# ryantd/tf-operator

Measured on AMD Instinct MI355X. Metric: samples/sec (1-worker TFJob), higher is better.
Workload: dtype bf16

## Files before the change

### csrc/hip/optim.hip

```cpp
#include "toa_common.h"

#include <algorithm>

template <bool BF16>
__global__ __launch_bounds__(256) void sumsq_partial_kernel(const void* __restrict__ x, int64_t n,
                                                            float* __restrict__ partial) {
  __shared__ float red[4];
  float acc = 0.f;
  const int64_t n8 = n / 8;
  for (int64_t i = blockIdx.x * (int64_t)blockDim.x + threadIdx.x; i < n8;
       i += (int64_t)gridDim.x * blockDim.x) {
    float f[8];
    if (BF16) {
      unpack8(ld16((const bf16_t*)x + i * 8), f);
    } else {
      f32x4 a = *((const f32x4*)x + 2 * i), b = *((const f32x4*)x + 2 * i + 1);
      f[0] = a[0]; f[1] = a[1]; f[2] = a[2]; f[3] = a[3];
      f[4] = b[0]; f[5] = b[1]; f[6] = b[2]; f[7] = b[3];
    }
#pragma unroll
    for (int j = 0; j < 8; ++j) acc = fmaf(f[j], f[j], acc);
  }
  if (blockIdx.x == 0) {
    for (int64_t i = n8 * 8 + threadIdx.x; i < n; i += blockDim.x) {
// ... 150 lines not shown
  const float ns = norm_sq[0];
  const bool bad = (__float_as_uint(ns) & 0x7f800000u) == 0x7f800000u;
  const int f = (bad || (limit > 0.f && sqrtf(ns) * grad_scale > limit)) ? 1 : 0;
  flag[0] = f;
  skipped[0] += f;
}

extern "C" int toa_adamw_guard(const float* norm_sq, float grad_scale, float limit, int* flag, int* skipped,
                               hipStream_t stream) {
  if (norm_sq == nullptr || flag == nullptr || skipped == nullptr) return (int)hipErrorInvalidValue;
  hipLaunchKernelGGL(adamw_guard_kernel, dim3(1), dim3(1), 0, stream, norm_sq, grad_scale, limit, flag, skipped);
  return (int)hipGetLastError();
}

__device__ __forceinline__ int guard_step(int step, const int* skipped, float b1, float b2, float& inv_bc1,
                                          float& inv_sqrt_bc2) {
  const int sk = skipped[0];
  if (sk != 0) {
    const float st = (float)(step - sk);
    inv_bc1 = 1.f / (1.f - powf(b1, st));
    inv_sqrt_bc2 = 1.f / sqrtf(1.f - powf(b2, st));
  }
  return step - sk;
}

template <bool GRAD_BF16, bool NT, typename MT = float, bool GUARD = false>
__global__ __launch_bounds__(256) void adamw_flat_kernel(float* __restrict__ master, bf16_t* __restrict__ param,
                                                         void* __restrict__ grad, int zero_grad, MT* __restrict__ m,
                                                         MT* __restrict__ v, int64_t n8, float lr, float b1,
                                                         float b2, float eps, float wd, float inv_bc1,
                                                         float inv_sqrt_bc2, float grad_scale,
                                                         const float* __restrict__ norm_sq, float max_norm,
                                                         const int* __restrict__ step_dev, int step, int64_t base,
                                                         uint32_t seed, const int* __restrict__ flag,
                                                         const int* __restrict__ skipped) {
  constexpr bool MB = sizeof(MT) == 2;
  if constexpr (GUARD) {
    if (flag[0] != 0) {
      if (zero_grad) {
        const int64_t nz = GRAD_BF16 ? n8 : 2 * n8;
        for (int64_t i = blockIdx.x * (int64_t)blockDim.x + threadIdx.x; i < nz; i += (int64_t)gridDim.x * blockDim.x)
          *((u32x4*)grad + i) = u32x4{0, 0, 0, 0};
      }
      return;
    }
    step = guard_step(step, skipped, b1, b2, inv_bc1, inv_sqrt_bc2);
  }
  const float scale = adam_prologue(b1, b2, grad_scale, norm_sq, max_norm, step_dev, inv_bc1, inv_sqrt_bc2);
  const float omb1 = 1.f - b1, omb2 = 1.f - b2, lrwd = lr * wd;
  const uint32_t key = MB ? sr_key(step_dev != nullptr ? step_dev[0] : step, seed) : 0u;
  for (int64_t i = blockIdx.x * (int64_t)blockDim.x + threadIdx.x; i < n8;
       i += (int64_t)gridDim.x * blockDim.x) {
    float g[8], p[8], mm[8], vv[8];
    if (GRAD_BF16) {
      unpack8(ld_s((const u32x4*)grad + i, NT), g);
      if (zero_grad) st16((bf16_t*)grad + i * 8, u32x4{0, 0, 0, 0});
    } else {
      f32x4 a = ld_s((const f32x4*)grad + 2 * i, NT), b = ld_s((const f32x4*)grad + 2 * i + 1, NT);
      g[0] = a[0]; g[1] = a[1]; g[2] = a[2]; g[3] = a[3];
      g[4] = b[0]; g[5] = b[1]; g[6] = b[2]; g[7] = b[3];
      if (zero_grad) {
        *((f32x4*)grad + 2 * i) = f32x4{0.f, 0.f, 0.f, 0.f};
        *((f32x4*)grad + 2 * i + 1) = f32x4{0.f, 0.f, 0.f, 0.f};
      }
    }
    f32x4* pm = (f32x4*)master + 2 * i;
    f32x4 p0 = ld_s(pm, NT), p1 = ld_s(pm + 1, NT);
    if constexpr (MB) {
      u32x4* mv = (u32x4*)m + i;
      u32x4* vvp = (u32x4*)v + i;
      const u32x4 mb = ld_s(mv, NT), vb = ld_s(vvp, NT);
      unpack8(mb, mm);
      unpack8(vb, vv);
#pragma unroll
      for (int j = 0; j < 4; ++j) {
        p[j] = p0[j]; p[j + 4] = p1[j];
      }
#pragma unroll
      for (int j = 0; j < 8; ++j)
        adam_elem(g[j], p[j], mm[j], vv[j], scale, b1, b2, omb1, omb2, lr, lrwd, eps, inv_bc1, inv_sqrt_bc2);
#pragma unroll
      for (int j = 0; j < 4; ++j) {
        p0[j] = p[j]; p1[j] = p[j + 4];
      }
      u32x4 mo, vo;
      sr_pack8(mm, vv, base + 8 * i, key, mo, vo);
      st_s(pm, p0, NT); st_s(pm + 1, p1, NT);
      st_s(mv, mo, NT);
      st_s(vvp, vo, NT);
    } else {
      f32x4* mv = (f32x4*)m + 2 * i;
      f32x4* vvp = (f32x4*)v + 2 * i;
      f32x4 m0 = ld_s(mv, NT), m1 = ld_s(mv + 1, NT), v0 = ld_s(vvp, NT), v1 = ld_s(vvp + 1, NT);
#pragma unroll
      for (int j = 0; j < 4; ++j) {
        p[j] = p0[j]; p[j + 4] = p1[j];
        mm[j] = m0[j]; mm[j + 4] = m1[j];
        vv[j] = v0[j]; vv[j + 4] = v1[j];
      }
#pragma unroll
      for (int j = 0; j < 8; ++j)
        adam_elem(g[j], p[j], mm[j], vv[j], scale, b1, b2, omb1, omb2, lr, lrwd, eps, inv_bc1, inv_sqrt_bc2);
#pragma unroll
      for (int j = 0; j < 4; ++j) {
        p0[j] = p[j]; p1[j] = p[j + 4];
        m0[j] = mm[j]; m1[j] = mm[j + 4];
        v0[j] = vv[j]; v1[j] = vv[j + 4];
      }
      st_s(pm, p0, NT); st_s(pm + 1, p1, NT);
      st_s(mv, m0, NT); st_s(mv + 1, m1, NT);
      st_s(vvp, v0, NT); st_s(vvp + 1, v1, NT);
    }
    if (param != nullptr) st_s((u32x4*)param + i, pack8(p), NT);
  }
}

template <typename MT = float, bool GUARD = false>
__global__ __launch_bounds__(256) void adamw_wt_kernel(float* __restrict__ master, bf16_t* __restrict__ param,
                                                       bf16_t* __restrict__ grad, int zero_grad,
                                                       MT* __restrict__ m, MT* __restrict__ v,
                                                       bf16_t* __restrict__ wt, int64_t ldt, int R, int C, float lr,
                                                       float b1, float b2, float eps, float wd, float inv_bc1,
                                                       float inv_sqrt_bc2, float grad_scale,
                                                       const float* __restrict__ norm_sq, float max_norm, int step,
                                                       int64_t base, uint32_t seed, const int* __restrict__ flag,
                                                       const int* __restrict__ skipped) {
  constexpr bool MB = sizeof(MT) == 2;
  __shared__ u32x4 tile[128 * 16];
  if constexpr (GUARD) {
    if (flag[0] != 0) {
      if (zero_grad) {
        const int64_t nz = (int64_t)R * C / 8;
        for (int64_t i = blockIdx.x * (int64_t)blockDim.x + threadIdx.x; i < nz; i += (int64_t)gridDim.x * blockDim.x)
          st16(grad + i * 8, u32x4{0, 0, 0, 0});
      }
      return;
    }
    step = guard_step(step, skipped, b1, b2, inv_bc1, inv_sqrt_bc2);
  }
  const float scale = adam_prologue(b1, b2, grad_scale, norm_sq, max_norm, nullptr, inv_bc1, inv_sqrt_bc2);
  const float omb1 = 1.f - b1, omb2 = 1.f - b2, lrwd = lr * wd;
  const uint32_t key = MB ? sr_key(step, seed) : 0u;
  const int tid = threadIdx.x;
  const int lr_ = tid >> 4, lc = tid & 15;
  const int a = tid & 15, bq = tid >> 4;
  const int tiles_c = C >> 7;
  const int64_t ntiles = (int64_t)(R >> 7) * tiles_c;
  for (int64_t t = blockIdx.x; t < ntiles; t += gridDim.x) {
    const int tr = (int)(t / tiles_c), tc = (int)(t - (int64_t)tr * tiles_c);
    const int64_t r0 = (int64_t)tr * 128, c0 = (int64_t)tc * 128;
    __syncthreads();
#pragma unroll 1
    for (int pp = 0; pp < 8; pp += 2) {
      u32x4 gb[2], mb[2], vb[2];
      f32x4 pv[2][2], mv[2][2], vv[2][2];
      int64_t e8[2];
#pragma unroll
      for (int q = 0; q < 2; ++q) {
        const int r = lr_ + 16 * (pp + q);
        e8[q] = ((r0 + r) * C + c0) / 8 + lc;
        gb[q] = ld_s((const u32x4*)grad + e8[q], true);
        pv[q][0] = ld_s((const f32x4*)master + 2 * e8[q], true);
        pv[q][1] = ld_s((const f32x4*)master + 2 * e8[q] + 1, true);
        if constexpr (MB) {
          mb[q] = ld_s((const u32x4*)m + e8[q], true);
          vb[q] = ld_s((const u32x4*)v + e8[q], true);
        } else {
          mv[q][0] = ld_s((const f32x4*)m + 2 * e8[q], true);
          mv[q][1] = ld_s((const f32x4*)m + 2 * e8[q] + 1, true);
          vv[q][0] = ld_s((const f32x4*)v + 2 * e8[q], true);
          vv[q][1] = ld_s((const f32x4*)v + 2 * e8[q] + 1, true);
        }
      }
#pragma unroll
      for (int q = 0; q < 2; ++q) {
        const int r = lr_ + 16 * (pp + q);
        float g[8], p[8];
        unpack8(gb[q], g);
        if (zero_grad) st16(grad + e8[q] * 8, u32x4{0, 0, 0, 0});
        if constexpr (MB) {
          float t[8];
          unpack8(mb[q], t);
          mv[q][0] = f32x4{t[0], t[1], t[2], t[3]};
          mv[q][1] = f32x4{t[4], t[5], t[6], t[7]};
          unpack8(vb[q], t);
          vv[q][0] = f32x4{t[0], t[1], t[2], t[3]};
          vv[q][1] = f32x4{t[4], t[5], t[6], t[7]};
        }
#pragma unroll
        for (int h = 0; h < 2; ++h)
#pragma unroll
          for (int j = 0; j < 4; ++j) {
            float pp_ = pv[q][h][j], mm = mv[q][h][j], vq = vv[q][h][j];
            adam_elem(g[4 * h + j], pp_, mm, vq, scale, b1, b2, omb1, omb2, lr, lrwd, eps, inv_bc1, inv_sqrt_bc2);
            pv[q][h][j] = pp_;
            mv[q][h][j] = mm;
            vv[q][h][j] = vq;
            p[4 * h + j] = pp_;
          }
        st_s((f32x4*)master + 2 * e8[q], pv[q][0], true);
        st_s((f32x4*)master + 2 * e8[q] + 1, pv[q][1], true);
        if constexpr (MB) {
          const float mf[8] = {mv[q][0][0], mv[q][0][1], mv[q][0][2], mv[q][0][3],
                               mv[q][1][0], mv[q][1][1], mv[q][1][2], mv[q][1][3]};
          const float vf[8] = {vv[q][0][0], vv[q][0][1], vv[q][0][2], vv[q][0][3],
                               vv[q][1][0], vv[q][1][1], vv[q][1][2], vv[q][1][3]};
          u32x4 mo, vo;
          sr_pack8(mf, vf, base + 8 * e8[q], key, mo, vo);
          st_s((u32x4*)m + e8[q], mo, true);
          st_s((u32x4*)v + e8[q], vo, true);
        } else {
          st_s((f32x4*)m + 2 * e8[q], mv[q][0], true);
          st_s((f32x4*)m + 2 * e8[q] + 1, mv[q][1], true);
          st_s((f32x4*)v + 2 * e8[q], vv[q][0], true);
          st_s((f32x4*)v + 2 * e8[q] + 1, vv[q][1], true);
        }
        const u32x4 pk = pack8(p);
        st_s((u32x4*)param + e8[q], pk, true);
        tile[r * 16 + (lc ^ ((r >> 3) & 15))] = pk;
      }
    }
    __syncthreads();
    u32x4 in[8], out[8];
#pragma unroll
    for (int i = 0; i < 8; ++i) in[i] = tile[(8 * a + i) * 16 + (bq ^ a)];
    tr8x8(in, out);
    bf16_t* d = wt + (c0 + 8 * bq) * ldt + r0 + 8 * a;
#pragma unroll
    for (int j = 0; j < 8; ++j) __builtin_nontemporal_store(out[j], (u32x4*)(d + j * ldt));
  }
}

template <typename MT, bool GUARD = false>
static int adamw_wt_launch(float* master, bf16_t* param, bf16_t* grad, int zero_grad, MT* m, MT* v, bf16_t* wt,
                           int64_t ldt, int R, int C, float lr, float beta1, float beta2, float eps,
                           float weight_decay, int step, float grad_scale, const float* norm_sq, float max_norm,
                           int64_t base, uint32_t seed, hipStream_t stream, const int* flag = nullptr,
                           const int* skipped = nullptr) {
  if (GUARD && (flag == nullptr || skipped == nullptr)) return (int)hipErrorInvalidValue;
  if (R <= 0 || C <= 0 || R % 128 || C % 128 || ldt < R || ldt % 8 || ((uintptr_t)master & 15) ||
      ((uintptr_t)m & 15) || ((uintptr_t)v & 15) || ((uintptr_t)grad & 15) || ((uintptr_t)param & 15) ||
      ((uintptr_t)wt & 15) || step < 1 || base < 0 || base % 8)
    return (int)hipErrorInvalidValue;
  const float inv_bc1 = 1.f / (1.f - powf(beta1, (float)step));
  const float inv_sqrt_bc2 = 1.f / sqrtf(1.f - powf(beta2, (float)step));
  const int64_t tiles = (int64_t)(R / 128) * (C / 128);
  const int grid = (int)(tiles < 16384 ? tiles : 16384);
  hipLaunchKernelGGL((adamw_wt_kernel<MT, GUARD>), dim3(grid), dim3(256), 0, stream, master, param, grad, zero_grad,
                     m, v, wt, ldt, R, C, lr, beta1, beta2, eps, weight_decay, inv_bc1, inv_sqrt_bc2, grad_scale,
                     norm_sq, max_norm, step, base, seed, flag, skipped);
  return (int)hipGetLastError();
}

// ... 104 lines not shown
  return adamw_launch<bf16_t, true>(master, param, grad, grad_flags, m, v, n, lr, beta1, beta2, eps, weight_decay,
                                    step, grad_scale, norm_sq, max_norm, nullptr, base, seed, stream, flag, skipped);
}

extern "C" int toa_adamw_flat_bf16s_dstep(float* master, bf16_t* param, void* grad, int grad_flags, bf16_t* m,
                                          bf16_t* v, int64_t n, float lr, float beta1, float beta2, float eps,
                                          float weight_decay, const int* step_dev, float grad_scale,
                                          const float* norm_sq, float max_norm, int64_t base, uint32_t seed,
                                          hipStream_t stream) {
  if (!bf16s_args_ok(master, param, grad, m, v, n, base) || step_dev == nullptr) return (int)hipErrorInvalidValue;
  return adamw_launch(master, param, grad, grad_flags, m, v, n, lr, beta1, beta2, eps, weight_decay, 1, grad_scale,
                      norm_sq, max_norm, step_dev, base, seed, stream);
}

extern "C" int toa_adamw_flat_dstep(float* master, bf16_t* param, void* grad, int grad_flags, float* m, float* v,
                                    int64_t n, float lr, float beta1, float beta2, float eps, float weight_decay,
                                    const int* step_dev, float grad_scale, const float* norm_sq, float max_norm,
                                    hipStream_t stream) {
  if (step_dev == nullptr) return (int)hipErrorInvalidValue;
  return adamw_launch(master, param, grad, grad_flags, m, v, n, lr, beta1, beta2, eps, weight_decay, 1, grad_scale,
                      norm_sq, max_norm, step_dev, 0, 0u, stream);
}

__global__ void step_inc_kernel(int* step) { step[0] += 1; }

extern "C" int toa_step_inc(int* step, hipStream_t stream) {
  hipLaunchKernelGGL(step_inc_kernel, dim3(1), dim3(1), 0, stream, step);
  return (int)hipGetLastError();
}

__global__ __launch_bounds__(256) void sgd_flat_kernel(float* __restrict__ p, const float* __restrict__ g,
                                                       float* __restrict__ buf, int64_t n, float lr,
                                                       float momentum, float wd) {
  for (int64_t i = blockIdx.x * (int64_t)blockDim.x + threadIdx.x; i < n; i += (int64_t)gridDim.x * blockDim.x) {
    float gi = g[i] + wd * p[i];
    if (buf != nullptr) {
      float b = momentum * buf[i] + gi;
      buf[i] = b;
      gi = b;
    }
    p[i] -= lr * gi;
  }
}

extern "C" int toa_sgd_flat(float* p, const float* g, float* momentum_buf, int64_t n, float lr, float momentum,
                            float weight_decay, hipStream_t stream) {
// ... 46 lines not shown
```

### tf_operator_amd/ops/_lib.py

```python
from __future__ import annotations

import ctypes
import os
import threading

import torch

_HERE = os.path.dirname(os.path.abspath(__file__))
LIB_PATH = os.environ.get("TOA_HIP_LIB") or os.path.join(os.path.dirname(_HERE), "lib", "libtoa_hip.so")

_lock = threading.Lock()
_lib = None
_err = None

c_int = ctypes.c_int
c_i64 = ctypes.c_int64
c_f = ctypes.c_float
c_p = ctypes.c_void_p

_SIGS = {
    "toa_sumsq": [c_p, c_i64, c_int, c_p, c_p, c_int, c_p],
    "toa_adamw_flat": [c_p, c_p, c_p, c_int, c_p, c_p, c_i64, c_f, c_f, c_f, c_f, c_f, c_int, c_f, c_p, c_f, c_p],
    "toa_adamw_flat_dstep": [c_p, c_p, c_p, c_int, c_p, c_p, c_i64, c_f, c_f, c_f, c_f, c_f, c_p, c_f, c_p, c_f,
                             c_p],
    "toa_adamw_flat_bf16s": [c_p, c_p, c_p, c_int, c_p, c_p, c_i64, c_f, c_f, c_f, c_f, c_f, c_int, c_f, c_p, c_f,
                             c_i64, ctypes.c_uint32, c_p],
    "toa_adamw_flat_bf16s_dstep": [c_p, c_p, c_p, c_int, c_p, c_p, c_i64, c_f, c_f, c_f, c_f, c_f, c_p, c_f, c_p, c_f,
                                   c_i64, ctypes.c_uint32, c_p],
    "toa_adamw_wt_bf16s": [c_p, c_p, c_p, c_int, c_p, c_p, c_p, c_i64, c_int, c_int, c_f, c_f, c_f, c_f, c_f, c_int,
                           c_f, c_p, c_f, c_i64, ctypes.c_uint32, c_p],
    "toa_adamw_guard": [c_p, c_f, c_f, c_p, c_p, c_p],
    "toa_adamw_flat_guard": [c_p, c_p, c_p, c_int, c_p, c_p, c_i64, c_f, c_f, c_f, c_f, c_f, c_int, c_f, c_p, c_f,
                             c_p, c_p, c_p],
    "toa_adamw_flat_bf16s_guard": [c_p, c_p, c_p, c_int, c_p, c_p, c_i64, c_f, c_f, c_f, c_f, c_f, c_int, c_f, c_p, c_f,
                                   c_i64, ctypes.c_uint32, c_p, c_p, c_p],
    "toa_adamw_wt_guard": [c_p, c_p, c_p, c_int, c_p, c_p, c_p, c_i64, c_int, c_int, c_f, c_f, c_f, c_f, c_f, c_int,
                           c_f, c_p, c_f, c_p, c_p, c_p],
    "toa_adamw_wt_bf16s_guard": [c_p, c_p, c_p, c_int, c_p, c_p, c_p, c_i64, c_int, c_int, c_f, c_f, c_f, c_f, c_f,
                                 c_int, c_f, c_p, c_f, c_i64, ctypes.c_uint32, c_p, c_p, c_p],
    "toa_norm_set_fwd_cap": [c_int],
    "toa_lastline_arm": [ctypes.c_char_p, c_i64, c_i64, c_int],
    "toa_lastline_disarm": [],
    "toa_gemm_asm_set_swiglu_persist": [c_int],
    "toa_xent_set_unroll": [c_int],
    "toa_transpose_set_variant": [c_int],
    "toa_wgrad_asm_set_sumsq": [c_p],
    "toa_sum_f32": [c_p, c_i64, c_p, c_p, c_int, c_p],
    "toa_sumsq_ranges": [c_p, c_p, c_p, c_int, c_p, c_p, c_int, c_p],
    "toa_gemm_asm_rope": [c_p, c_i64, c_p, c_i64, c_p, c_p, c_int, c_int, c_int, c_int, c_int, c_p],
    "toa_gemm_asm_delta": [c_p, c_i64, c_p, c_i64, c_p, c_i64, c_p, c_p, c_int, c_int, c_int, c_int, c_int, c_p],
    "toa_gemm_asm_resadd": [c_p, c_i64, c_p, c_i64, c_p, c_i64, c_p, c_int, c_int, c_int, c_p],
    "toa_gemm_nn_asm": [c_p, c_i64, c_p, c_i64, c_p, c_i64, c_int, c_int, c_int, c_p],
    "toa_gemm_nn_asm_swiglu_bwd": [c_p, c_i64, c_p, c_i64, c_p, c_i64, c_p, c_i64, c_int, c_int, c_int, c_p],
    "toa_gemm_nn_asm_delta": [c_p, c_i64, c_p, c_i64, c_p, c_i64, c_p, c_p, c_int, c_int, c_int, c_int, c_int, c_p],
    "toa_adamw_wt": [c_p, c_p, c_p, c_int, c_p, c_p, c_p, c_i64, c_int, c_int, c_f, c_f, c_f, c_f, c_f, c_int, c_f,
                     c_p, c_f, c_p],
    "toa_stream_create_cu_mask": [c_int, c_int, ctypes.POINTER(ctypes.c_void_p)],
    "toa_stream_destroy": [c_p],
    "toa_step_inc": [c_p, c_p],
    "toa_set_stream_variant": [c_int],
    "toa_sgd_flat": [c_p, c_p, c_p, c_i64, c_f, c_f, c_f, c_p],
    "toa_cast_f32_to_bf16": [c_p, c_p, c_i64, c_p],
# ... 229 lines not shown
```

### tf_operator_amd/ops/optim.py

```python
from __future__ import annotations

import ctypes
import math
import os

import torch

from . import _lib
from .wt import transpose_into


SUMSQ_WS = 32768


def grad_norm_sq(flat_grad: torch.Tensor, workspace=None, out=None):
    out = torch.zeros(1, device=flat_grad.device, dtype=torch.float32) if out is None else out
    if _lib.use_hip(flat_grad):
        ws = torch.empty(SUMSQ_WS, device=flat_grad.device, dtype=torch.float32) if workspace is None else workspace
        _lib.call("toa_sumsq", _lib.ptr(flat_grad), flat_grad.numel(), int(flat_grad.dtype == torch.bfloat16),
                  _lib.ptr(ws), _lib.ptr(out), 0, _lib.stream(flat_grad))
    else:
        out.copy_(flat_grad.float().pow(2).sum().reshape(1))
    return out

# ... 54 lines not shown
    if m.dtype == torch.bfloat16:
        m, v = m.float(), v.float()
    m.mul_(beta1).add_(g, alpha=1 - beta1)
    v.mul_(beta2).addcmul_(g, g, value=1 - beta2)
    bc1 = 1 - beta1 ** step
    bc2 = 1 - beta2 ** step
    denom = v.sqrt() / math.sqrt(bc2) + eps
    master.add_(-lr * (m / bc1) / denom - lr * weight_decay * master)
    if m_out is not m:
        mb, vb = sr_round_moments(m, v, base, step, seed)
        m_out.copy_(mb)
        v_out.copy_(vb)


def check_skip_limit(skip_nonfinite: bool, skip_grad_norm) -> float:
    limit = float(skip_grad_norm or 0.0)
    if not math.isfinite(limit) or limit < 0:
        raise ValueError(f"skip_grad_norm must be a finite number >= 0, not {skip_grad_norm!r}")
    if limit > 0 and not skip_nonfinite:
        raise ValueError("skip_grad_norm needs skip_nonfinite: the limit is part of the skipped-step guard")
    return limit


_MASKED = []


def masked_stream(n: int, mode: int = 1, device=None):
    h = ctypes.c_void_p()
    _lib.call("toa_stream_create_cu_mask", int(mode), int(n), ctypes.byref(h))
    st = torch.cuda.ExternalStream(h.value, device=device)
    _MASKED.append((st, h))
    return st


class FlatAdamW:

    def __init__(self, flat, lr=3e-4, betas=(0.9, 0.95), eps=1e-8, weight_decay=0.1, max_grad_norm=1.0,
                 overlap=False, buckets=None, fuse_zero_grad=False, post_update=None, owned=None, group=None,
                 device_step=False, state_dtype=torch.float32, seed=0, skip_nonfinite=False, skip_grad_norm=0.0):
        if state_dtype not in (torch.float32, torch.bfloat16):
            raise ValueError(f"state_dtype must be torch.float32 or torch.bfloat16, not {state_dtype!r}")
        self.skip_nonfinite = bool(skip_nonfinite)
        self.skip_grad_norm = check_skip_limit(self.skip_nonfinite, skip_grad_norm)
        if self.skip_nonfinite and device_step:
            raise ValueError("skip_nonfinite: the device-step (graph-replayed) update has no guarded form")
        self._flag = torch.zeros(1, device=flat.device, dtype=torch.int32) if self.skip_nonfinite else None
        self._skipped = torch.zeros(1, device=flat.device, dtype=torch.int32) if self.skip_nonfinite else None
        self.state_dtype = state_dtype
        self.seed = int(seed) & _U32
        self.post_update = post_update
        self.sumsq = None
        self.fused_wt = None
        self.device_step = (bool(device_step) and flat.device.type == "cuda" and _lib.available()
                            and _lib.has("toa_adamw_flat_dstep"))
        self._dstep = torch.zeros(1, device=flat.device, dtype=torch.int32) if self.device_step else None
        self.owned = None if owned is None else [tuple(r) for r in owned]
        self.group = group
        if self.owned is not None and overlap:
            raise ValueError("overlap mode and a sharded update are exclusive")
        self.flat = flat
        self.lr = lr
        self.beta1, self.beta2 = betas
        self.eps = eps
        self.weight_decay = weight_decay
        self.max_grad_norm = max_grad_norm
        self.step_count = 0
        flat.moment_dtype, flat.moment_seed = state_dtype, self.seed
        if flat.exp_avg is None:
            flat.exp_avg = torch.zeros(flat.state_numel, device=flat.device, dtype=state_dtype)
            flat.exp_avg_sq = torch.zeros(flat.state_numel, device=flat.device, dtype=state_dtype)
        self._convert_moments()
        self.runs = flat.decay_runs() if weight_decay else [[0, flat.numel, False]]
        self._norm = torch.zeros(1, device=flat.device, dtype=torch.float32)
        self._ws = torch.empty(SUMSQ_WS, device=flat.device, dtype=torch.float32)
        self.last_norm_sq = self._norm
# ... 62 lines not shown
            return {}
        out = {}
        for a, b, p, view in wt.items:
            R, C = p.shape
            if R % 128 == 0 and C % 128 == 0 and f.state_index(b - 1) == f.state_index(a) + (b - a - 1):
                out[(a, b)] = (a, b, p, view)
        return out

    def _launch_wt(self, item, decay, lr, grad_scale, clip, stream):
        a, b, p, view = item
        f = self.flat
        si = f.state_index(a)
        R, C = p.shape
        bf = self._bf16_state()
        es = f.exp_avg.element_size()
        fn, tail = self._guarded("toa_adamw_wt_bf16s" if bf else "toa_adamw_wt", (a, self.seed) if bf else (), stream)
        _lib.call(fn, f.master.data_ptr() + 4 * si,
                  f.param.data_ptr() + 2 * a,
                  f.grad.data_ptr() + 2 * a, int(bool(self.fuse_zero_grad)), f.exp_avg.data_ptr() + es * si,
                  f.exp_avg_sq.data_ptr() + es * si, _lib.ptr(view), view.stride(0), R, C, float(lr),
                  float(self.beta1), float(self.beta2), float(self.eps), float(self.weight_decay if decay else 0.0),
                  self.step_count, float(grad_scale), _lib.ptr(self._norm) if clip else None,
                  float(self.max_grad_norm or 0.0), *tail)

    def _work_runs(self):
        if self.owned is None:
            yield from self.runs
            return
        for lo, hi in self.owned:
            for a, b, decay in self.runs:
                a2, b2 = max(a, lo), min(b, hi)
                if a2 < b2:
                    yield a2, b2, decay

    def _norm_sq(self):
        f = self.flat
        if self.owned is None:
            if self.sumsq is not None:
                self.sumsq.norm_sq(self._norm, self._ws)
                return
            grad_norm_sq(f.grad, self._ws, self._norm)
            return
        import torch.distributed as dist

        if _lib.use_hip(f.grad):
            for i, (lo, hi) in enumerate(self.owned):
# ... 60 lines not shown
                    if a2 < b2:
                        self._launch(a2, b2, decay, lr, grad_scale, clip, self.fuse_zero_grad, s)
                if self.post_update is not None:
                    with torch.cuda.stream(self.side):
                        self.post_update(lo, hi)
                ev = torch.cuda.Event()
                ev.record(self.side)
                self.events[bi] = ev
                self.waited[bi] = False
            self.done = torch.cuda.Event()
            self.done.record(self.side)
            for t in (f.grad, f.param, f.master, f.exp_avg, f.exp_avg_sq, self._norm, self._flag, self._skipped):
                if t is not None:
                    t.record_stream(self.side)
            self.grads_zeroed = self.fuse_zero_grad
            return
        self.grads_zeroed = False
        if _lib.use_hip(f.grad):
            s = _lib.stream(f.grad)
            pbf = f.param.dtype == torch.bfloat16
            if self.device_step:
                _lib.call("toa_step_inc", _lib.ptr(self._dstep), s)
            fused = self._fused_items() if pbf else {}
            for (a, b, decay) in self._work_runs():
                pos = a
                for ia, ib in sorted(k for k in fused if a <= k[0] and k[1] <= b):
                    if pos < ia:
                        self._launch(pos, ia, decay, lr, grad_scale, clip, self.fuse_zero_grad, s)
                    self._launch_wt(fused[(ia, ib)], decay, lr, grad_scale, clip, s)
                    pos = ib
                if pos < b:
                    self._launch(pos, b, decay, lr, grad_scale, clip, self.fuse_zero_grad, s)
            self.grads_zeroed = self.fuse_zero_grad and self.owned is None
            if not pbf:
                f.param_from_master()
            if fused:
                done = {id(it[2]) for it in fused.values()}
                for _, _, p, view in self.fused_wt.items:
                    if id(p) not in done:
                        transpose_into(view, p.data)
            elif self.post_update is not None:
                self.post_update(0, f.numel)
        else:
            st = self._host_step()
            for (a, b, decay) in (self._work_runs() if st else ()):
                adamw_reference(f.state_view(f.master, a, b), f.grad[a:b], f.state_view(f.exp_avg, a, b),
                                f.state_view(f.exp_avg_sq, a, b), lr=lr,
                                beta1=self.beta1, beta2=self.beta2, eps=self.eps,
                                weight_decay=self.weight_decay if decay else 0.0, step=st,
                                grad_scale=grad_scale, norm_sq=self._norm if clip else None,
                                max_norm=self.max_grad_norm or 0.0, base=a, seed=self.seed)
            for lo, hi in (self.owned or [(0, f.numel)]):
                f.param[lo:hi].copy_(f.state_view(f.master, lo, hi).to(f.param.dtype))
            if self.post_update is not None:
                self.post_update(0, f.numel)
# ... 84 lines not shown
```

Baseline: 6.600.

## Fuse all AdamW segment launches into a single segment-table kernel

Replaces the per-run sequence of flat and transpose-writing AdamW kernel launches with one kernel. That kernel walks a device-resident segment table, using a prefix-sum binary search to map each block's work unit to a flat chunk or a 128x128 transposed tile. The per-element and per-tile bodies are factored into shared device functions. The table is cached keyed on tensor pointers. The goal is to cut kernel launch and Python dispatch overhead and tail underutilisation across many small segments, at the cost of a per-unit lookup and possible imbalance between tile and flat units.

After: 6.618 (median of 6 runs). No clear change (+0.3%).

```diff
diff --git a/csrc/hip/adam_one.h b/csrc/hip/adam_one.h
--- /dev/null
+++ b/csrc/hip/adam_one.h
@@ -0,0 +1,62 @@
+#pragma once
+
+#include <stdint.h>
+
+#if defined(__HIPCC__)
+#define TOA_HD __host__ __device__
+#else
+#define TOA_HD
+#endif
+
+struct AdamSeg {
+  void* master;
+  void* param;
+  void* grad;
+  void* m;
+  void* v;
+  void* wt;
+  int64_t ldt;
+  int64_t base;
+  int64_t n;
+  int32_t R, C;
+  int32_t flags;
+  int32_t pad;
+};
+
+static_assert(sizeof(AdamSeg) == 88, "ops/optim.py AdamSeg mirrors this layout");
+
+enum { ADAM_SEG_WT = 1, ADAM_SEG_DECAY = 2, ADAM_SEG_NT = 4 };
+
+constexpr int64_t ADAM_ONE_FLAT_UNIT = 2048;
+constexpr int64_t ADAM_ONE_TILE = 128 * 128;
+
+static inline int adam_seg_check(const AdamSeg& s) {
+  const uintptr_t align = (uintptr_t)s.master | (uintptr_t)s.param | (uintptr_t)s.grad | (uintptr_t)s.m |
+                          (uintptr_t)s.v | (uintptr_t)s.wt;
+  if (s.master == nullptr || s.param == nullptr || s.grad == nullptr || s.m == nullptr || s.v == nullptr) return 1;
+  if (align & 15) return 2;
+  if (s.n <= 0 || s.n % 8) return 3;
+  if (s.base < 0 || s.base % 8) return 4;
+  if (s.flags & ~(ADAM_SEG_WT | ADAM_SEG_DECAY | ADAM_SEG_NT)) return 5;
+  if (s.flags & ADAM_SEG_WT) {
+    if (s.wt == nullptr || s.R <= 0 || s.C <= 0 || s.R % 128 || s.C % 128 || (int64_t)s.R * s.C != s.n) return 6;
+    if (s.ldt < s.R || s.ldt % 8) return 7;
+  }
+  return 0;
+}
+
+static inline int64_t adam_seg_units(const AdamSeg& s) {
+  return (s.flags & ADAM_SEG_WT) ? s.n / ADAM_ONE_TILE : (s.n + ADAM_ONE_FLAT_UNIT - 1) / ADAM_ONE_FLAT_UNIT;
+}
+
+TOA_HD static inline int adam_one_find(const int64_t* prefix, int nseg, int64_t u) {
+  int lo = 0, hi = nseg;
+  while (hi - lo > 1) {
+    const int mid = (lo + hi) >> 1;
+    if (prefix[mid] <= u)
+      lo = mid;
+    else
+      hi = mid;
+  }
+  return lo;
+}
diff --git a/csrc/hip/optim.hip b/csrc/hip/optim.hip
--- a/csrc/hip/optim.hip
+++ b/csrc/hip/optim.hip
@@ -1,4 +1,5 @@
 #include "toa_common.h"
+#include "adam_one.h"
 
 #include <algorithm>
 
@@ -196,6 +197,81 @@
     inv_sqrt_bc2 = 1.f / sqrtf(1.f - powf(b2, st));
   }
   return step - sk;
+}
+
+struct AdamK {
+  float scale, b1, b2, omb1, omb2, lr, lrwd, eps, inv_bc1, inv_sqrt_bc2;
+  uint32_t key;
+};
+
+template <bool GRAD_BF16, bool NT, typename MT>
+__device__ __forceinline__ void adam_flat_chunk(float* __restrict__ master, bf16_t* __restrict__ param,
+                                                void* __restrict__ grad, int zero_grad, MT* __restrict__ m,
+                                                MT* __restrict__ v, int64_t i, const AdamK& k, int64_t base) {
+  constexpr bool MB = sizeof(MT) == 2;
+  float g[8], p[8], mm[8], vv[8];
+  if (GRAD_BF16) {
+    unpack8(ld_s((const u32x4*)grad + i, NT), g);
+    if (zero_grad) st16((bf16_t*)grad + i * 8, u32x4{0, 0, 0, 0});
+  } else {
+    f32x4 a = ld_s((const f32x4*)grad + 2 * i, NT), b = ld_s((const f32x4*)grad + 2 * i + 1, NT);
+    g[0] = a[0]; g[1] = a[1]; g[2] = a[2]; g[3] = a[3];
+    g[4] = b[0]; g[5] = b[1]; g[6] = b[2]; g[7] = b[3];
+    if (zero_grad) {
+      *((f32x4*)grad + 2 * i) = f32x4{0.f, 0.f, 0.f, 0.f};
+      *((f32x4*)grad + 2 * i + 1) = f32x4{0.f, 0.f, 0.f, 0.f};
+    }
+  }
+  f32x4* pm = (f32x4*)master + 2 * i;
+  f32x4 p0 = ld_s(pm, NT), p1 = ld_s(pm + 1, NT);
+  if constexpr (MB) {
+    u32x4* mv = (u32x4*)m + i;
+    u32x4* vvp = (u32x4*)v + i;
+    const u32x4 mb = ld_s(mv, NT), vb = ld_s(vvp, NT);
+    unpack8(mb, mm);
+    unpack8(vb, vv);
+#pragma unroll
+    for (int j = 0; j < 4; ++j) {
+      p[j] = p0[j]; p[j + 4] = p1[j];
+    }
+#pragma unroll
+    for (int j = 0; j < 8; ++j)
+      adam_elem(g[j], p[j], mm[j], vv[j], k.scale, k.b1, k.b2, k.omb1, k.omb2, k.lr, k.lrwd, k.eps, k.inv_bc1,
+                k.inv_sqrt_bc2);
+#pragma unroll
+    for (int j = 0; j < 4; ++j) {
+      p0[j] = p[j]; p1[j] = p[j + 4];
+    }
+    u32x4 mo, vo;
+    sr_pack8(mm, vv, base + 8 * i, k.key, mo, vo);
+    st_s(pm, p0, NT); st_s(pm + 1, p1, NT);
+    st_s(mv, mo, NT);
+    st_s(vvp, vo, NT);
+  } else {
+    f32x4* mv = (f32x4*)m + 2 * i;
+    f32x4* vvp = (f32x4*)v + 2 * i;
+    f32x4 m0 = ld_s(mv, NT), m1 = ld_s(mv + 1, NT), v0 = ld_s(vvp, NT), v1 = ld_s(vvp + 1, NT);
+#pragma unroll
+    for (int j = 0; j < 4; ++j) {
+      p[j] = p0[j]; p[j + 4] = p1[j];
+      mm[j] = m0[j]; mm[j + 4] = m1[j];
+      vv[j] = v0[j]; vv[j + 4] = v1[j];
+    }
+#pragma unroll
+    for (int j = 0; j < 8; ++j)
+      adam_elem(g[j], p[j], mm[j], vv[j], k.scale, k.b1, k.b2, k.omb1, k.omb2, k.lr, k.lrwd, k.eps, k.inv_bc1,
+                k.inv_sqrt_bc2);
+#pragma unroll
+    for (int j = 0; j < 4; ++j) {
+      p0[j] = p[j]; p1[j] = p[j + 4];
+      m0[j] = mm[j]; m1[j] = mm[j + 4];
+      v0[j] = vv[j]; v1[j] = vv[j + 4];
+    }
+    st_s(pm, p0, NT); st_s(pm + 1, p1, NT);
+    st_s(mv, m0, NT); st_s(mv + 1, m1, NT);
+    st_s(vvp, v0, NT); st_s(vvp + 1, v1, NT);
+  }
+  if (param != nullptr) st_s((u32x4*)param + i, pack8(p), NT);
 }
 
 template <bool GRAD_BF16, bool NT, typename MT = float, bool GUARD = false>
@@ -223,70 +299,104 @@
   const float scale = adam_prologue(b1, b2, grad_scale, norm_sq, max_norm, step_dev, inv_bc1, inv_sqrt_bc2);
   const float omb1 = 1.f - b1, omb2 = 1.f - b2, lrwd = lr * wd;
   const uint32_t key = MB ? sr_key(step_dev != nullptr ? step_dev[0] : step, seed) : 0u;
+  const AdamK k{scale, b1, b2, omb1, omb2, lr, lrwd, eps, inv_bc1, inv_sqrt_bc2, key};
   for (int64_t i = blockIdx.x * (int64_t)blockDim.x + threadIdx.x; i < n8;
-       i += (int64_t)gridDim.x * blockDim.x) {
-    float g[8], p[8], mm[8], vv[8];
-    if (GRAD_BF16) {
-      unpack8(ld_s((const u32x4*)grad + i, NT), g);
-      if (zero_grad) st16((bf16_t*)grad + i * 8, u32x4{0, 0, 0, 0});
-    } else {
-      f32x4 a = ld_s((const f32x4*)grad + 2 * i, NT), b = ld_s((const f32x4*)grad + 2 * i + 1, NT);
-      g[0] = a[0]; g[1] = a[1]; g[2] = a[2]; g[3] = a[3];
-      g[4] = b[0]; g[5] = b[1]; g[6] = b[2]; g[7] = b[3];
-      if (zero_grad) {
-        *((f32x4*)grad + 2 * i) = f32x4{0.f, 0.f, 0.f, 0.f};
-        *((f32x4*)grad + 2 * i + 1) = f32x4{0.f, 0.f, 0.f, 0.f};
+       i += (int64_t)gridDim.x * blockDim.x)
+    adam_flat_chunk<GRAD_BF16, NT, MT>(master, param, grad, zero_grad, m, v, i, k, base);
+}
+
+template <typename MT>
+__device__ __forceinline__ void adam_wt_tile(float* __restrict__ master, bf16_t* __restrict__ param,
+                                             bf16_t* __restrict__ grad, int zero_grad, MT* __restrict__ m,
+                                             MT* __restrict__ v, bf16_t* __restrict__ wt, int64_t ldt, int C,
+                                             int64_t t, const AdamK& k, int64_t base, u32x4* tile) {
+  constexpr bool MB = sizeof(MT) == 2;
+  const int tid = threadIdx.x;
+  const int lr_ = tid >> 4, lc = tid & 15;
+  const int a = tid & 15, bq = tid >> 4;
+  const int tiles_c = C >> 7;
+  const int tr = (int)(t / tiles_c), tc = (int)(t - (int64_t)tr * tiles_c);
+  const int64_t r0 = (int64_t)tr * 128, c0 = (int64_t)tc * 128;
+  __syncthreads();
+#pragma unroll 1
+  for (int pp = 0; pp < 8; pp += 2) {
+    u32x4 gb[2], mb[2], vb[2];
+    f32x4 pv[2][2], mv[2][2], vv[2][2];
+    int64_t e8[2];
+#pragma unroll
+    for (int q = 0; q < 2; ++q) {
+      const int r = lr_ + 16 * (pp + q);
+      e8[q] = ((r0 + r) * C + c0) / 8 + lc;
+      gb[q] = ld_s((const u32x4*)grad + e8[q], true);
+      pv[q][0] = ld_s((const f32x4*)master + 2 * e8[q], true);
+      pv[q][1] = ld_s((const f32x4*)master + 2 * e8[q] + 1, true);
+      if constexpr (MB) {
+        mb[q] = ld_s((const u32x4*)m + e8[q], true);
+        vb[q] = ld_s((const u32x4*)v + e8[q], true);
+      } else {
+        mv[q][0] = ld_s((const f32x4*)m + 2 * e8[q], true);
+        mv[q][1] = ld_s((const f32x4*)m + 2 * e8[q] + 1, true);
+        vv[q][0] = ld_s((const f32x4*)v + 2 * e8[q], true);
+        vv[q][1] = ld_s((const f32x4*)v + 2 * e8[q] + 1, true);
       }
     }
-    f32x4* pm = (f32x4*)master + 2 * i;
-    f32x4 p0 = ld_s(pm, NT), p1 = ld_s(pm + 1, NT);
-    if constexpr (MB) {
-      u32x4* mv = (u32x4*)m + i;
-      u32x4* vvp = (u32x4*)v + i;
-      const u32x4 mb = ld_s(mv, NT), vb = ld_s(vvp, NT);
-      unpack8(mb, mm);
-      unpack8(vb, vv);
-#pragma unroll
-      for (int j = 0; j < 4; ++j) {
-        p[j] = p0[j]; p[j + 4] = p1[j];
+#pragma unroll
+    for (int q = 0; q < 2; ++q) {
+      const int r = lr_ + 16 * (pp + q);
+      float g[8], p[8];
+      unpack8(gb[q], g);
+      if (zero_grad) st16(grad + e8[q] * 8, u32x4{0, 0, 0, 0});
+      if constexpr (MB) {
+        float t[8];
+        unpack8(mb[q], t);
+        mv[q][0] = f32x4{t[0], t[1], t[2], t[3]};
+        mv[q][1] = f32x4{t[4], t[5], t[6], t[7]};
+        unpack8(vb[q], t);
+        vv[q][0] = f32x4{t[0], t[1], t[2], t[3]};
+        vv[q][1] = f32x4{t[4], t[5], t[6], t[7]};
       }
 #pragma unroll
-      for (int j = 0; j < 8; ++j)
-        adam_elem(g[j], p[j], mm[j], vv[j], scale, b1, b2, omb1, omb2, lr, lrwd, eps, inv_bc1, inv_sqrt_bc2);
-#pragma unroll
-      for (int j = 0; j < 4; ++j) {
-        p0[j] = p[j]; p1[j] = p[j + 4];
+      for (int h = 0; h < 2; ++h)
+#pragma unroll
+        for (int j = 0; j < 4; ++j) {
+          float pp_ = pv[q][h][j], mm = mv[q][h][j], vq = vv[q][h][j];
+          adam_elem(g[4 * h + j], pp_, mm, vq, k.scale, k.b1, k.b2, k.omb1, k.omb2, k.lr, k.lrwd, k.eps, k.inv_bc1,
+                    k.inv_sqrt_bc2);
+          pv[q][h][j] = pp_;
+          mv[q][h][j] = mm;
+          vv[q][h][j] = vq;
+          p[4 * h + j] = pp_;
+        }
+      st_s((f32x4*)master + 2 * e8[q], pv[q][0], true);
+      st_s((f32x4*)master + 2 * e8[q] + 1, pv[q][1], true);
+      if constexpr (MB) {
+        const float mf[8] = {mv[q][0][0], mv[q][0][1], mv[q][0][2], mv[q][0][3],
+                             mv[q][1][0], mv[q][1][1], mv[q][1][2], mv[q][1][3]};
+        const float vf[8] = {vv[q][0][0], vv[q][0][1], vv[q][0][2], vv[q][0][3],
+                             vv[q][1][0], vv[q][1][1], vv[q][1][2], vv[q][1][3]};
+        u32x4 mo, vo;
+        sr_pack8(mf, vf, base + 8 * e8[q], k.key, mo, vo);
+        st_s((u32x4*)m + e8[q], mo, true);
+        st_s((u32x4*)v + e8[q], vo, true);
+      } else {
+        st_s((f32x4*)m + 2 * e8[q], mv[q][0], true);
+        st_s((f32x4*)m + 2 * e8[q] + 1, mv[q][1], true);
+        st_s((f32x4*)v + 2 * e8[q], vv[q][0], true);
+        st_s((f32x4*)v + 2 * e8[q] + 1, vv[q][1], true);
       }
-      u32x4 mo, vo;
-      sr_pack8(mm, vv, base + 8 * i, key, mo, vo);
-      st_s(pm, p0, NT); st_s(pm + 1, p1, NT);
-      st_s(mv, mo, NT);
-      st_s(vvp, vo, NT);
-    } else {
-      f32x4* mv = (f32x4*)m + 2 * i;
-      f32x4* vvp = (f32x4*)v + 2 * i;
-      f32x4 m0 = ld_s(mv, NT), m1 = ld_s(mv + 1, NT), v0 = ld_s(vvp, NT), v1 = ld_s(vvp + 1, NT);
-#pragma unroll
-      for (int j = 0; j < 4; ++j) {
-        p[j] = p0[j]; p[j + 4] = p1[j];
-        mm[j] = m0[j]; mm[j + 4] = m1[j];
-        vv[j] = v0[j]; vv[j + 4] = v1[j];
-      }
-#pragma unroll
-      for (int j = 0; j < 8; ++j)
-        adam_elem(g[j], p[j], mm[j], vv[j], scale, b1, b2, omb1, omb2, lr, lrwd, eps, inv_bc1, inv_sqrt_bc2);
-#pragma unroll
-      for (int j = 0; j < 4; ++j) {
-        p0[j] = p[j]; p1[j] = p[j + 4];
-        m0[j] = mm[j]; m1[j] = mm[j + 4];
-        v0[j] = vv[j]; v1[j] = vv[j + 4];
-      }
-      st_s(pm, p0, NT); st_s(pm + 1, p1, NT);
-      st_s(mv, m0, NT); st_s(mv + 1, m1, NT);
-      st_s(vvp, v0, NT); st_s(vvp + 1, v1, NT);
-    }
-    if (param != nullptr) st_s((u32x4*)param + i, pack8(p), NT);
-  }
+      const u32x4 pk = pack8(p);
+      st_s((u32x4*)param + e8[q], pk, true);
+      tile[r * 16 + (lc ^ ((r >> 3) & 15))] = pk;
+    }
+  }
+  __syncthreads();
+  u32x4 in[8], out[8];
+#pragma unroll
+  for (int i = 0; i < 8; ++i) in[i] = tile[(8 * a + i) * 16 + (bq ^ a)];
+  tr8x8(in, out);
+  bf16_t* d = wt + (c0 + 8 * bq) * ldt + r0 + 8 * a;
+#pragma unroll
+  for (int j = 0; j < 8; ++j) __builtin_nontemporal_store(out[j], (u32x4*)(d + j * ldt));
 }
 
 template <typename MT = float, bool GUARD = false>
@@ -315,94 +425,10 @@
   const float scale = adam_prologue(b1, b2, grad_scale, norm_sq, max_norm, nullptr, inv_bc1, inv_sqrt_bc2);
   const float omb1 = 1.f - b1, omb2 = 1.f - b2, lrwd = lr * wd;
   const uint32_t key = MB ? sr_key(step, seed) : 0u;
-  const int tid = threadIdx.x;
-  const int lr_ = tid >> 4, lc = tid & 15;
-  const int a = tid & 15, bq = tid >> 4;
-  const int tiles_c = C >> 7;
-  const int64_t ntiles = (int64_t)(R >> 7) * tiles_c;
-  for (int64_t t = blockIdx.x; t < ntiles; t += gridDim.x) {
-    const int tr = (int)(t / tiles_c), tc = (int)(t - (int64_t)tr * tiles_c);
-    const int64_t r0 = (int64_t)tr * 128, c0 = (int64_t)tc * 128;
-    __syncthreads();
-#pragma unroll 1
-    for (int pp = 0; pp < 8; pp += 2) {
-      u32x4 gb[2], mb[2], vb[2];
-      f32x4 pv[2][2], mv[2][2], vv[2][2];
-      int64_t e8[2];
-#pragma unroll
-      for (int q = 0; q < 2; ++q) {
-        const int r = lr_ + 16 * (pp + q);
-        e8[q] = ((r0 + r) * C + c0) / 8 + lc;
-        gb[q] = ld_s((const u32x4*)grad + e8[q], true);
-        pv[q][0] = ld_s((const f32x4*)master + 2 * e8[q], true);
-        pv[q][1] = ld_s((const f32x4*)master + 2 * e8[q] + 1, true);
-        if constexpr (MB) {
-          mb[q] = ld_s((const u32x4*)m + e8[q], true);
-          vb[q] = ld_s((const u32x4*)v + e8[q], true);
-        } else {
-          mv[q][0] = ld_s((const f32x4*)m + 2 * e8[q], true);
-          mv[q][1] = ld_s((const f32x4*)m + 2 * e8[q] + 1, true);
-          vv[q][0] = ld_s((const f32x4*)v + 2 * e8[q], true);
-          vv[q][1] = ld_s((const f32x4*)v + 2 * e8[q] + 1, true);
-        }
-      }
-#pragma unroll
-      for (int q = 0; q < 2; ++q) {
-        const int r = lr_ + 16 * (pp + q);
-        float g[8], p[8];
-        unpack8(gb[q], g);
-        if (zero_grad) st16(grad + e8[q] * 8, u32x4{0, 0, 0, 0});
-        if constexpr (MB) {
-          float t[8];
-          unpack8(mb[q], t);
-          mv[q][0] = f32x4{t[0], t[1], t[2], t[3]};
-          mv[q][1] = f32x4{t[4], t[5], t[6], t[7]};
-          unpack8(vb[q], t);
-          vv[q][0] = f32x4{t[0], t[1], t[2], t[3]};
-          vv[q][1] = f32x4{t[4], t[5], t[6], t[7]};
-        }
-#pragma unroll
-        for (int h = 0; h < 2; ++h)
-#pragma unroll
-          for (int j = 0; j < 4; ++j) {
-            float pp_ = pv[q][h][j], mm = mv[q][h][j], vq = vv[q][h][j];
-            adam_elem(g[4 * h + j], pp_, mm, vq, scale, b1, b2, omb1, omb2, lr, lrwd, eps, inv_bc1, inv_sqrt_bc2);
-            pv[q][h][j] = pp_;
-            mv[q][h][j] = mm;
-            vv[q][h][j] = vq;
-            p[4 * h + j] = pp_;
-          }
-        st_s((f32x4*)master + 2 * e8[q], pv[q][0], true);
-        st_s((f32x4*)master + 2 * e8[q] + 1, pv[q][1], true);
-        if constexpr (MB) {
-          const float mf[8] = {mv[q][0][0], mv[q][0][1], mv[q][0][2], mv[q][0][3],
-                               mv[q][1][0], mv[q][1][1], mv[q][1][2], mv[q][1][3]};
-          const float vf[8] = {vv[q][0][0], vv[q][0][1], vv[q][0][2], vv[q][0][3],
-                               vv[q][1][0], vv[q][1][1], vv[q][1][2], vv[q][1][3]};
-          u32x4 mo, vo;
-          sr_pack8(mf, vf, base + 8 * e8[q], key, mo, vo);
-          st_s((u32x4*)m + e8[q], mo, true);
-          st_s((u32x4*)v + e8[q], vo, true);
-        } else {
-          st_s((f32x4*)m + 2 * e8[q], mv[q][0], true);
-          st_s((f32x4*)m + 2 * e8[q] + 1, mv[q][1], true);
-          st_s((f32x4*)v + 2 * e8[q], vv[q][0], true);
-          st_s((f32x4*)v + 2 * e8[q] + 1, vv[q][1], true);
-        }
-        const u32x4 pk = pack8(p);
-        st_s((u32x4*)param + e8[q], pk, true);
-        tile[r * 16 + (lc ^ ((r >> 3) & 15))] = pk;
-      }
-    }
-    __syncthreads();
-    u32x4 in[8], out[8];
-#pragma unroll
-    for (int i = 0; i < 8; ++i) in[i] = tile[(8 * a + i) * 16 + (bq ^ a)];
-    tr8x8(in, out);
-    bf16_t* d = wt + (c0 + 8 * bq) * ldt + r0 + 8 * a;
-#pragma unroll
-    for (int j = 0; j < 8; ++j) __builtin_nontemporal_store(out[j], (u32x4*)(d + j * ldt));
-  }
+  const AdamK k{scale, b1, b2, omb1, omb2, lr, lrwd, eps, inv_bc1, inv_sqrt_bc2, key};
+  const int64_t ntiles = (int64_t)(R >> 7) * (C >> 7);
+  for (int64_t t = blockIdx.x; t < ntiles; t += gridDim.x)
+    adam_wt_tile<MT>(master, param, grad, zero_grad, m, v, wt, ldt, C, t, k, base, tile);
 }
 
 template <typename MT, bool GUARD = false>
@@ -553,6 +579,105 @@
                       norm_sq, max_norm, step_dev, 0, 0u, stream);
 }
 
+template <typename MT, bool GUARD>
+__global__ __launch_bounds__(256) void adamw_one_kernel(const AdamSeg* __restrict__ segs,
+                                                        const int64_t* __restrict__ prefix, int nseg, int64_t total,
+                                                        int zero_grad, float lr, float b1, float b2, float eps,
+                                                        float wd, float inv_bc1, float inv_sqrt_bc2, float grad_scale,
+                                                        const float* __restrict__ norm_sq, float max_norm, int step,
+                                                        uint32_t seed, const int* __restrict__ flag,
+                                                        const int* __restrict__ skipped) {
+  constexpr bool MB = sizeof(MT) == 2;
+  __shared__ u32x4 tile[128 * 16];
+  if constexpr (GUARD) {
+    if (flag[0] != 0) {
+      if (zero_grad) {
+        for (int64_t u = blockIdx.x; u < total; u += gridDim.x) {
+          const int si = adam_one_find(prefix, nseg, u);
+          const AdamSeg& sg = segs[si];
+          const int64_t per = (sg.flags & ADAM_SEG_WT) ? ADAM_ONE_TILE / 8 : ADAM_ONE_FLAT_UNIT / 8;
+          const int64_t c0 = (u - prefix[si]) * per, c1 = c0 + per < sg.n / 8 ? c0 + per : sg.n / 8;
+          for (int64_t i = c0 + threadIdx.x; i < c1; i += blockDim.x)
+            st16((bf16_t*)sg.grad + i * 8, u32x4{0, 0, 0, 0});
+        }
+      }
+      return;
+    }
+    step = guard_step(step, skipped, b1, b2, inv_bc1, inv_sqrt_bc2);
+  }
+  const float scale = adam_prologue(b1, b2, grad_scale, norm_sq, max_norm, nullptr, inv_bc1, inv_sqrt_bc2);
+  const float omb1 = 1.f - b1, omb2 = 1.f - b2;
+  const uint32_t key = MB ? sr_key(step, seed) : 0u;
+  for (int64_t u = blockIdx.x; u < total; u += gridDim.x) {
+    const int si = adam_one_find(prefix, nseg, u);
+    const AdamSeg& sg = segs[si];
+    const int64_t lu = u - prefix[si];
+    const int flags = sg.flags;
+    const AdamK k{scale, b1, b2, omb1, omb2, lr, lr * ((flags & ADAM_SEG_DECAY) ? wd : 0.f), eps, inv_bc1,
+                  inv_sqrt_bc2, key};
+    if (flags & ADAM_SEG_WT) {
+      adam_wt_tile<MT>((float*)sg.master, (bf16_t*)sg.param, (bf16_t*)sg.grad, zero_grad, (MT*)sg.m, (MT*)sg.v,
+                       (bf16_t*)sg.wt, sg.ldt, sg.C, lu, k, sg.base, tile);
+    } else {
+      const int64_t i = lu * (ADAM_ONE_FLAT_UNIT / 8) + threadIdx.x;
+      if (i < sg.n / 8) {
+        if (flags & ADAM_SEG_NT)
+          adam_flat_chunk<true, true, MT>((float*)sg.master, (bf16_t*)sg.param, sg.grad, zero_grad, (MT*)sg.m,
+                                          (MT*)sg.v, i, k, sg.base);
+        else
+          adam_flat_chunk<true, false, MT>((float*)sg.master, (bf16_t*)sg.param, sg.grad, zero_grad, (MT*)sg.m,
+                                           (MT*)sg.v, i, k, sg.base);
+      }
+    }
+  }
+}
+
+extern "C" int toa_adam_one_build(AdamSeg* segs, int nseg, int64_t* prefix) {
+  if (segs == nullptr || prefix == nullptr || nseg <= 0) return (int)hipErrorInvalidValue;
+  int64_t units = 0;
+  for (int i = 0; i < nseg; ++i) {
+    if (adam_seg_check(segs[i]) != 0) return (int)hipErrorInvalidValue;
+    if (!(segs[i].flags & ADAM_SEG_WT)) {
+      const bool nt = (g_stream_variant & 1) && segs[i].n / 8 >= (int64_t)(1 << 20);
+      segs[i].flags = (segs[i].flags & ~ADAM_SEG_NT) | (nt ? ADAM_SEG_NT : 0);
+    }
+    prefix[i] = units;
+    units += adam_seg_units(segs[i]);
+  }
+  prefix[nseg] = units;
+  return 0;
+}
+
+extern "C" int toa_adam_one_find(const int64_t* prefix, int nseg, int64_t u) {
+  if (prefix == nullptr || nseg <= 0 || u < 0 || u >= prefix[nseg]) return -1;
+  return adam_one_find(prefix, nseg, u);
+}
+
+static int g_adam_one_cap = 1 << 20;
+extern "C" int toa_adam_one_set_cap(int cap) {
+  const int old = g_adam_one_cap;
+  if (cap > 0) g_adam_one_cap = cap;
+  return old;
+}
+
+extern "C" int toa_adamw_one(const AdamSeg* segs, const int64_t* prefix, int nseg, int64_t total, int moments_bf16,
+                             int zero_grad, float lr, float beta1, float beta2, float eps, float weight_decay,
+                             int step, float grad_scale, const float* norm_sq, float max_norm, uint32_t seed,
+                             const int* flag, const int* skipped, hipStream_t stream) {
+  if (segs == nullptr || prefix == nullptr || nseg <= 0 || total < nseg || step < 1 ||
+      (flag == nullptr) != (skipped == nullptr))
+    return (int)hipErrorInvalidValue;
+  const float inv_bc1 = 1.f / (1.f - powf(beta1, (float)step));
+  const float inv_sqrt_bc2 = 1.f / sqrtf(1.f - powf(beta2, (float)step));
+  const int grid = (int)std::min<int64_t>(total, g_adam_one_cap);
+  const bool guard = flag != nullptr;
+  auto k = moments_bf16 ? (guard ? adamw_one_kernel<bf16_t, true> : adamw_one_kernel<bf16_t, false>)
+                        : (guard ? adamw_one_kernel<float, true> : adamw_one_kernel<float, false>);
+  hipLaunchKernelGGL(k, dim3(grid), dim3(256), 0, stream, segs, prefix, nseg, total, zero_grad, lr, beta1, beta2, eps,
+                     weight_decay, inv_bc1, inv_sqrt_bc2, grad_scale, norm_sq, max_norm, step, seed, flag, skipped);
+  return (int)hipGetLastError();
+}
+
 __global__ void step_inc_kernel(int* step) { step[0] += 1; }
 
 extern "C" int toa_step_inc(int* step, hipStream_t stream) {
diff --git a/tf_operator_amd/ops/_lib.py b/tf_operator_amd/ops/_lib.py
--- a/tf_operator_amd/ops/_lib.py
+++ b/tf_operator_amd/ops/_lib.py
@@ -38,6 +38,11 @@
                            c_f, c_p, c_f, c_p, c_p, c_p],
     "toa_adamw_wt_bf16s_guard": [c_p, c_p, c_p, c_int, c_p, c_p, c_p, c_i64, c_int, c_int, c_f, c_f, c_f, c_f, c_f,
                                  c_int, c_f, c_p, c_f, c_i64, ctypes.c_uint32, c_p, c_p, c_p],
+    "toa_adam_one_build": [c_p, c_int, c_p],
+    "toa_adam_one_find": [c_p, c_int, c_i64],
+    "toa_adam_one_set_cap": [c_int],
+    "toa_adamw_one": [c_p, c_p, c_int, c_i64, c_int, c_int, c_f, c_f, c_f, c_f, c_f, c_int, c_f, c_p, c_f,
+                      ctypes.c_uint32, c_p, c_p, c_p],
     "toa_norm_set_fwd_cap": [c_int],
     "toa_lastline_arm": [ctypes.c_char_p, c_i64, c_i64, c_int],
     "toa_lastline_disarm": [],
diff --git a/tf_operator_amd/ops/optim.py b/tf_operator_amd/ops/optim.py
--- a/tf_operator_amd/ops/optim.py
+++ b/tf_operator_amd/ops/optim.py
@@ -100,6 +100,37 @@
     return limit
 
 
+class AdamSeg(ctypes.Structure):
+    _fields_ = [("master", ctypes.c_void_p), ("param", ctypes.c_void_p), ("grad", ctypes.c_void_p),
+                ("m", ctypes.c_void_p), ("v", ctypes.c_void_p), ("wt", ctypes.c_void_p), ("ldt", ctypes.c_int64),
+                ("base", ctypes.c_int64), ("n", ctypes.c_int64), ("R", ctypes.c_int32), ("C", ctypes.c_int32),
+                ("flags", ctypes.c_int32), ("pad", ctypes.c_int32)]
+
+
+SEG_WT, SEG_DECAY = 1, 2
+ONE_FLAT_UNIT, ONE_TILE = 2048, 128 * 128
+
+
+def adam_one_prefix(segs):
+    out = [0]
+    for n, is_wt in segs:
+        out.append(out[-1] + (n // ONE_TILE if is_wt else -(-n // ONE_FLAT_UNIT)))
+    return out
+
+
+class AdamOneTable:
+
+    def __init__(self, segs, device):
+        arr = (AdamSeg * len(segs))(*segs)
+        prefix = (ctypes.c_int64 * (len(segs) + 1))()
+        _lib.call("toa_adam_one_build", arr, len(segs), prefix)
+        self.nseg = len(segs)
+        self.prefix_host = list(prefix)
+        self.total = self.prefix_host[-1]
+        self.segs = torch.frombuffer(bytearray(bytes(arr)), dtype=torch.uint8).to(device)
+        self.prefix = torch.tensor(self.prefix_host, dtype=torch.int64, device=device)
+
+
 _MASKED = []
 
 
@@ -129,6 +160,11 @@
         self.post_update = post_update
         self.sumsq = None
         self.fused_wt = None
+        env = os.environ.get("TOA_ADAM_ONE", "1")
+        if env not in ("0", "1"):
+            raise ValueError(f"TOA_ADAM_ONE must be 0 or 1, not {env!r}")
+        self.one_launch = env == "1"
+        self._one = self._one_key = None
         self.device_step = (bool(device_step) and flat.device.type == "cuda" and _lib.available()
                             and _lib.has("toa_adamw_flat_dstep"))
         self._dstep = torch.zeros(1, device=flat.device, dtype=torch.int32) if self.device_step else None
@@ -237,6 +273,50 @@
                   float(self.beta1), float(self.beta2), float(self.eps), float(self.weight_decay if decay else 0.0),
                   self.step_count, float(grad_scale), _lib.ptr(self._norm) if clip else None,
                   float(self.max_grad_norm or 0.0), *tail)
+
+    def _pieces(self, fused):
+        for (a, b, decay) in self._work_runs():
+            pos = a
+            for ia, ib in sorted(k for k in fused if a <= k[0] and k[1] <= b):
+                if pos < ia:
+                    yield pos, ia, decay, None
+                yield ia, ib, decay, fused[(ia, ib)]
+                pos = ib
+            if pos < b:
+                yield pos, b, decay, None
+
+    def _one_table(self, fused):
+        f = self.flat
+        key = (f.master.data_ptr(), f.param.data_ptr(), f.grad.data_ptr(), f.exp_avg.data_ptr(),
+               f.exp_avg_sq.data_ptr(), f.exp_avg.dtype,
+               tuple((a, b, it[3].data_ptr(), it[3].stride(0)) for (a, b), it in sorted(fused.items())))
+        if self._one is not None and key == self._one_key:
+            return self._one
+        es = f.exp_avg.element_size()
+        segs = []
+        for a, b, decay, item in self._pieces(fused):
+            si = f.state_index(a)
+            if f.state_index(b - 1) != si + (b - a - 1):
+                raise ValueError(f"update run [{a}, {b}) crosses fp32 state ranges")
+            seg = AdamSeg(master=f.master.data_ptr() + 4 * si, param=f.param.data_ptr() + 2 * a,
+                          grad=f.grad.data_ptr() + 2 * a, m=f.exp_avg.data_ptr() + es * si,
+                          v=f.exp_avg_sq.data_ptr() + es * si, base=a, n=b - a, flags=SEG_DECAY if decay else 0)
+            if item is not None:
+                view = item[3]
+                seg.wt, seg.ldt = view.data_ptr(), view.stride(0)
+                seg.R, seg.C = item[2].shape
+                seg.flags |= SEG_WT
+            segs.append(seg)
+        self._one, self._one_key = AdamOneTable(segs, f.device), key
+        return self._one
+
+    def _step_one(self, fused, lr, grad_scale, clip, stream):
+        t = self._one_table(fused)
+        guard = (_lib.ptr(self._flag), _lib.ptr(self._skipped)) if self.skip_nonfinite else (None, None)
+        _lib.call("toa_adamw_one", _lib.ptr(t.segs), _lib.ptr(t.prefix), t.nseg, t.total, int(self._bf16_state()),
+                  int(bool(self.fuse_zero_grad)), float(lr), float(self.beta1), float(self.beta2), float(self.eps),
+                  float(self.weight_decay), self.step_count, float(grad_scale),
+                  _lib.ptr(self._norm) if clip else None, float(self.max_grad_norm or 0.0), self.seed, *guard, stream)
 
     def _work_runs(self):
         if self.owned is None:
@@ -343,15 +423,15 @@
             if self.device_step:
                 _lib.call("toa_step_inc", _lib.ptr(self._dstep), s)
             fused = self._fused_items() if pbf else {}
-            for (a, b, decay) in self._work_runs():
-                pos = a
-                for ia, ib in sorted(k for k in fused if a <= k[0] and k[1] <= b):
-                    if pos < ia:
-                        self._launch(pos, ia, decay, lr, grad_scale, clip, self.fuse_zero_grad, s)
-                    self._launch_wt(fused[(ia, ib)], decay, lr, grad_scale, clip, s)
-                    pos = ib
-                if pos < b:
-                    self._launch(pos, b, decay, lr, grad_scale, clip, self.fuse_zero_grad, s)
+            if (self.one_launch and pbf and self.owned is None and not self.device_step
+                    and f.grad.dtype == torch.bfloat16 and _lib.has("toa_adamw_one")):
+                self._step_one(fused, lr, grad_scale, clip, s)
+            else:
+                for a, b, decay, item in self._pieces(fused):
+                    if item is None:
+                        self._launch(a, b, decay, lr, grad_scale, clip, self.fuse_zero_grad, s)
+                    else:
+                        self._launch_wt(item, decay, lr, grad_scale, clip, s)
             self.grads_zeroed = self.fuse_zero_grad and self.owned is None
             if not pbf:
                 f.param_from_master()
```
